# PolarisRisingWar/rgb-experiment

Measured on AMD Instinct MI355X. Metric: aggregated edges/sec (full-graph GCN d=128, reference epoch = train fwd+bwd+Adam + 2 eval fwd), higher is better.
Workload: dtype f32

## Files before the change

rgb_experiment_amd/csrc/gemm.hip:

```cpp
#include "rgbx_common.h"

namespace rgbx {
namespace {

constexpr int BM = 128, BN = 128, KT = 32;
enum { A_PLAIN = 0, A_BN = 1, A_ROWS = 2 };

struct TnExtra {
  const float* X;
  int64_t ldx;
  const float *mean, *rstd, *ca, *cb, *ck;
  const int32_t* rows;
  int64_t n_rows;
};
using f32x16 = __attribute__((ext_vector_type(16))) float;

template <int W>
__device__ __forceinline__ void stage_tile(float* __restrict__ lds, const float* __restrict__ src,
                                           int64_t ld, int64_t k0, int64_t k_end, int c0, int ncols) {
  const int tid = threadIdx.x;
#pragma unroll 4
  for (int p = 0; p < KT * W / 256; ++p) {
    const int idx = p * 256 + tid;
    const int r = idx / W, c = idx % W;
    const int64_t k = k0 + r;
    lds[r * W + c] = (k < k_end && c0 + c < ncols) ? src[k * ld + c0 + c] : 0.f;
  }
}

template <int W>
__device__ __forceinline__ void fetch_tile(float4 (&regs)[KT * (W / 4) / 256], const float* __restrict__ src, int64_t ld,
                                           int64_t k0, int64_t k_end, int c0, int ncols) {
#pragma unroll
  for (int p = 0; p < KT * (W / 4) / 256; ++p) {
    const int idx = p * 256 + threadIdx.x;
    const int r = idx / (W / 4), c = (idx % (W / 4)) * 4;
    const int64_t k = k0 + r;
    regs[p] = make_float4(0.f, 0.f, 0.f, 0.f);
    if (k < k_end && c0 + c < ncols) regs[p] = *reinterpret_cast<const float4*>(src + k * ld + c0 + c);
  }
}

template <int W>
__device__ __forceinline__ void put_tile(float* __restrict__ lds, const float4 (&regs)[KT * (W / 4) / 256]) {
#pragma unroll
  for (int p = 0; p < KT * (W / 4) / 256; ++p) {
    const int idx = p * 256 + threadIdx.x;
    const int r = idx / (W / 4), c = (idx % (W / 4)) * 4;
    *reinterpret_cast<float4*>(lds + r * W + c) = regs[p];
  }
}

template <int W>
__device__ __forceinline__ void put_tile_bn(float* __restrict__ lds, const float4 (&rg)[KT * (W / 4) / 256],
                                            const float4 (&rx)[KT * (W / 4) / 256], const float* __restrict__ lc,
                                            int64_t k0, int64_t k_end, int c0, int ncols) {
#pragma unroll
  for (int p = 0; p < KT * (W / 4) / 256; ++p) {
    const int idx = p * 256 + threadIdx.x;
    const int r = idx / (W / 4), c = (idx % (W / 4)) * 4;
    float4 v = rg[p];
    if (k0 + r < k_end && c0 + c < ncols) {
      const float4 mu = *reinterpret_cast<const float4*>(lc + 0 * W + c);
      const float4 rs = *reinterpret_cast<const float4*>(lc + 1 * W + c);
      const float4 a = *reinterpret_cast<const float4*>(lc + 2 * W + c);
      const float4 b = *reinterpret_cast<const float4*>(lc + 3 * W + c);
      const float4 k = *reinterpret_cast<const float4*>(lc + 4 * W + c);
      v.x = bn_bwd_input_grad(v.x, rx[p].x, mu.x, rs.x, a.x, b.x, k.x);
      v.y = bn_bwd_input_grad(v.y, rx[p].y, mu.y, rs.y, a.y, b.y, k.y);
      v.z = bn_bwd_input_grad(v.z, rx[p].z, mu.z, rs.z, a.z, b.z, k.z);
      v.w = bn_bwd_input_grad(v.w, rx[p].w, mu.w, rs.w, a.w, b.w, k.w);
    }
    *reinterpret_cast<float4*>(lds + r * W + c) = v;
  }
}

template <int W>
__device__ __forceinline__ void fetch_row_ids(int32_t (&ids)[KT * (W / 4) / 256], const int32_t* __restrict__ rows,
                                              int64_t j0, int64_t j_end) {
#pragma unroll
  for (int p = 0; p < KT * (W / 4) / 256; ++p) {
    const int64_t j = j0 + (p * 256 + (int)threadIdx.x) / (W / 4);
    ids[p] = j < j_end ? rows[j] : -1;
  }
}

template <int W>
__device__ __forceinline__ void fetch_tile_rows(float4 (&regs)[KT * (W / 4) / 256], const float* __restrict__ src,
                                                int64_t ld, const int32_t (&ids)[KT * (W / 4) / 256], int c0, int ncols) {
#pragma unroll
  for (int p = 0; p < KT * (W / 4) / 256; ++p) {
    const int c = ((p * 256 + (int)threadIdx.x) % (W / 4)) * 4;
    regs[p] = make_float4(0.f, 0.f, 0.f, 0.f);
    if (ids[p] >= 0 && c0 + c < ncols) regs[p] = *reinterpret_cast<const float4*>(src + (int64_t)ids[p] * ld + c0 + c);
  }
}

__device__ __forceinline__ int64_t lower_bound_rows(const int32_t* __restrict__ rows, int64_t n, int64_t key) {
  int64_t lo = 0, hi = n;
  while (lo < hi) {
    const int64_t mid = (lo + hi) >> 1;
    if (rows[mid] < key) lo = mid + 1; else hi = mid;
  }
  return lo;
}

template <bool VEC4, int MT, int MODE = A_PLAIN>
__global__ void __launch_bounds__(256)
gemm_tn_partial_kernel(const float* __restrict__ A, int64_t lda, const float* __restrict__ B, int64_t ldb,
                       float* __restrict__ part, float* __restrict__ colpart, int64_t K, int M, int N,
                       int64_t slab, TnExtra ex) {
  static_assert(MODE == A_PLAIN || VEC4, "the A_BN / A_ROWS forms exist on the 16-byte path only");
  constexpr int MI = MT / 64;
  __shared__ float lds[KT * (MT + 128) + (MODE == A_BN ? 5 * MT : 0)];
  float* la = lds;
  float* lb = lds + KT * MT;
  const int split = blockIdx.x;
  const int m0 = blockIdx.y * MT, n0 = blockIdx.z * BN;
  const int64_t k_begin = (int64_t)split * slab;
  const int64_t k_end = k_begin + slab < K ? k_begin + slab : K;
  const int wave = threadIdx.x >> 6, lane = threadIdx.x & 63;
  const int wm = (wave >> 1) * (MT / 2), wn = (wave & 1) * 64;
  const int kr = lane >> 5, cc = lane & 31;

  f32x16 acc[MI][2];
#pragma unroll
  for (int i = 0; i < MI; ++i)
#pragma unroll
    for (int j = 0; j < 2; ++j)
#pragma unroll
      for (int r = 0; r < 16; ++r) acc[i][j][r] = 0.f;

  const bool sums = colpart != nullptr && blockIdx.z == 0 && threadIdx.x < MT;
  float csum = 0.f;
  auto consume = [&]() {
    if (sums) {
#pragma unroll 8
      for (int r = 0; r < KT; ++r) csum += la[r * MT + threadIdx.x];
    }
#pragma unroll 4
    for (int kk = 0; kk < KT; kk += 2) {
      float a[MI];
#pragma unroll
      for (int i = 0; i < MI; ++i) a[i] = la[(kk + kr) * MT + wm + i * 32 + cc];
      const float b0 = lb[(kk + kr) * 128 + wn + cc];
      const float b1 = lb[(kk + kr) * 128 + wn + 32 + cc];
#pragma unroll
      for (int i = 0; i < MI; ++i) {
        acc[i][0] = __builtin_amdgcn_mfma_f32_32x32x2f32(a[i], b0, acc[i][0], 0, 0, 0);
        acc[i][1] = __builtin_amdgcn_mfma_f32_32x32x2f32(a[i], b1, acc[i][1], 0, 0, 0);
      }
    }
  };
  if constexpr (MODE == A_BN) {
    float* lc = lds + KT * (MT + 128);
    for (int i = threadIdx.x; i < 5 * MT; i += 256) {
      const float* src = i < MT ? ex.mean : i < 2 * MT ? ex.rstd : i < 3 * MT ? ex.ca : i < 4 * MT ? ex.cb : ex.ck;
      const int c = m0 + i % MT;
      lc[i] = c < M ? src[c] : 0.f;
    }
    float4 ra[KT * (MT / 4) / 256], rx[KT * (MT / 4) / 256], rb[KT * 32 / 256];
    fetch_tile<MT>(ra, A, lda, k_begin, k_end, m0, M);
    fetch_tile<MT>(rx, ex.X, ex.ldx, k_begin, k_end, m0, M);
    fetch_tile<128>(rb, B, ldb, k_begin, k_end, n0, N);
    for (int64_t k0 = k_begin; k0 < k_end; k0 += KT) {
      __syncthreads();
      put_tile_bn<MT>(la, ra, rx, lc, k0, k_end, m0, M);
      put_tile<128>(lb, rb);
      __syncthreads();
      if (k0 + KT < k_end) {
        fetch_tile<MT>(ra, A, lda, k0 + KT, k_end, m0, M);
        fetch_tile<MT>(rx, ex.X, ex.ldx, k0 + KT, k_end, m0, M);
        fetch_tile<128>(rb, B, ldb, k0 + KT, k_end, n0, N);
      }
      consume();
    }
  } else if constexpr (MODE == A_ROWS) {
    const int64_t j_begin = lower_bound_rows(ex.rows, ex.n_rows, k_begin);
    const int64_t j_end = lower_bound_rows(ex.rows, ex.n_rows, k_end);
    float4 ra[KT * (MT / 4) / 256], rb[KT * 32 / 256];
    int32_t ia[KT * (MT / 4) / 256], ib[KT * 32 / 256];
    fetch_row_ids<MT>(ia, ex.rows, j_begin, j_end);
    fetch_row_ids<128>(ib, ex.rows, j_begin, j_end);
    fetch_tile_rows<MT>(ra, A, lda, ia, m0, M);
    fetch_tile_rows<128>(rb, B, ldb, ib, n0, N);
    fetch_row_ids<MT>(ia, ex.rows, j_begin + KT, j_end);
    fetch_row_ids<128>(ib, ex.rows, j_begin + KT, j_end);
    for (int64_t j0 = j_begin; j0 < j_end; j0 += KT) {
      __syncthreads();
      put_tile<MT>(la, ra);
      put_tile<128>(lb, rb);
      __syncthreads();
      if (j0 + KT < j_end) {
        fetch_tile_rows<MT>(ra, A, lda, ia, m0, M);
        fetch_tile_rows<128>(rb, B, ldb, ib, n0, N);
        fetch_row_ids<MT>(ia, ex.rows, j0 + 2 * KT, j_end);
        fetch_row_ids<128>(ib, ex.rows, j0 + 2 * KT, j_end);
      }
      consume();
    }
  } else if constexpr (VEC4) {
    float4 ra[KT * (MT / 4) / 256], rb[KT * 32 / 256];
    fetch_tile<MT>(ra, A, lda, k_begin, k_end, m0, M);
    fetch_tile<128>(rb, B, ldb, k_begin, k_end, n0, N);
    for (int64_t k0 = k_begin; k0 < k_end; k0 += KT) {
      __syncthreads();
      put_tile<MT>(la, ra);
      put_tile<128>(lb, rb);
      __syncthreads();
      if (k0 + KT < k_end) {
        fetch_tile<MT>(ra, A, lda, k0 + KT, k_end, m0, M);
        fetch_tile<128>(rb, B, ldb, k0 + KT, k_end, n0, N);
      }
      consume();
    }
  } else {
    for (int64_t k0 = k_begin; k0 < k_end; k0 += KT) {
      __syncthreads();
      stage_tile<MT>(la, A, lda, k0, k_end, m0, M);
      stage_tile<128>(lb, B, ldb, k0, k_end, n0, N);
      __syncthreads();
      consume();
    }
  }

  if (sums && m0 + (int)threadIdx.x < M) colpart[(int64_t)split * M + m0 + threadIdx.x] = csum;
  float* out = part + (int64_t)split * M * N;
#pragma unroll
  for (int i = 0; i < MI; ++i)
#pragma unroll
    for (int j = 0; j < 2; ++j)
#pragma unroll
      for (int r = 0; r < 16; ++r) {
        const int m = m0 + wm + i * 32 + (r & 3) + 8 * (r >> 2) + 4 * kr;
        const int n = n0 + wn + j * 32 + cc;
        if (m < M && n < N) out[(int64_t)m * N + n] = acc[i][j][r];
      }
}

__global__ void __launch_bounds__(256)
gemm_tn_reduce_kernel(const float* __restrict__ part, int S, int64_t MN, float* __restrict__ C, int N,
                      int64_t ldc, float alpha) {
  __shared__ float sh[8][32];
  const int j = threadIdx.x & 31, q = threadIdx.x >> 5;
  for (int64_t base = (int64_t)blockIdx.x * 32; base < MN; base += (int64_t)gridDim.x * 32) {
    const int64_t i = base + j;
    float s = 0.f;
    if (i < MN)
      for (int p = q; p < S; p += 8) s += part[(int64_t)p * MN + i];
    __syncthreads();
    sh[q][j] = s;
    __syncthreads();
    if (q == 0 && i < MN) {
      float t = 0.f;
#pragma unroll
      for (int k = 0; k < 8; ++k) t += sh[k][j];
      C[(i / N) * ldc + (i % N)] = alpha * t;
    }
  }
}

int tile_rows(int M) { return M <= 64 ? 64 : BM; }

int choose_splits(int64_t K, int M, int N) {
  const int64_t tiles = cdiv(M, tile_rows(M)) * cdiv(N, BN);
  int64_t s = cdiv(tile_rows(M) == 64 ? 1024 : 768, tiles);
  const int64_t max_s = cdiv(K, 16 * KT);
  if (s > max_s) s = max_s;
  if (s < 1) s = 1;
  return (int)s;
}

}
}

using namespace rgbx;

extern "C" int rgbx_gemm_tn_workspace_bytes(int64_t K, int64_t M, int64_t N, size_t* bytes) {
  if (!bytes || K < 0 || M < 0 || N < 0) return fail(RGBX_E_ARG, "gemm_tn_workspace_bytes: bad argument");
  if (M >= INT32_MAX || N >= INT32_MAX) return fail(RGBX_E_RANGE, "gemm_tn: M or N exceeds int32");
  *bytes = (size_t)choose_splits(K, (int)M, (int)N) * ((size_t)M * (size_t)N + (size_t)M) * sizeof(float);
  return RGBX_OK;
}

namespace rgbx {
namespace {

int run_gemm_tn(const char* name, int mode, const float* A, int64_t lda, const float* B, int64_t ldb, float* C,
                int64_t ldc, float* a_colsum, int64_t K, int64_t M, int64_t N, float alpha, void* workspace,
                size_t workspace_bytes, rgbx_stream_t stream, const TnExtra& ex) {
  if (K < 0 || M < 0 || N < 0) return fail(RGBX_E_ARG, "%s: negative size", name);
  if (M == 0 || N == 0) return RGBX_OK;
  if (!C || (K > 0 && (!A || !B))) return fail(RGBX_E_ARG, "%s: null pointer", name);
  if (M >= INT32_MAX || N >= INT32_MAX) return fail(RGBX_E_RANGE, "%s: M or N exceeds int32", name);
  if (lda < M || ldb < N || ldc < N) return fail(RGBX_E_ARG, "%s: leading dimension too small", name);
  bool v4 = aligned16(A) && aligned16(B) && lda % 4 == 0 && ldb % 4 == 0;
  if (mode == A_BN) {
    if (K > 0 && (!ex.X || !ex.mean || !ex.rstd || !ex.ca || !ex.cb || !ex.ck))
      return fail(RGBX_E_ARG, "%s: null pointer", name);
    if (ex.ldx < M) return fail(RGBX_E_ARG, "%s: leading dimension too small", name);
    v4 = v4 && aligned16(ex.X) && ex.ldx % 4 == 0;
  }
  if (mode == A_ROWS) {
    if (ex.n_rows < 0 || ex.n_rows > K || (ex.n_rows > 0 && !ex.rows)) return fail(RGBX_E_ARG, "%s: bad row list", name);
    if (K >= INT32_MAX) return fail(RGBX_E_RANGE, "%s: K exceeds int32", name);
  }
  if (mode != A_PLAIN && !v4)
    return fail(RGBX_E_ALIGN, "%s: operands must be 16-byte aligned with leading dimensions that are multiples of 4", name);
  size_t need = 0;
  if (int rc = rgbx_gemm_tn_workspace_bytes(K, M, N, &need)) return rc;
  if (!workspace || workspace_bytes < need)
    return fail(RGBX_E_WS, "%s: workspace %zu < %zu bytes", name, workspace_bytes, need);
  hipStream_t s = (hipStream_t)stream;
  const int S = choose_splits(K, (int)M, (int)N);
  const int64_t slab = cdiv(cdiv(K > 0 ? K : 1, S), KT) * KT;
  float* part = static_cast<float*>(workspace);
  float* colpart = a_colsum ? part + (size_t)S * M * N : nullptr;
  const int mt = tile_rows((int)M);
  dim3 grid(S, (unsigned)cdiv(M, mt), (unsigned)cdiv(N, BN));
#define RGBX_GEMM_TN(V4, MT, MODE) \
  gemm_tn_partial_kernel<V4, MT, MODE><<<grid, 256, 0, s>>>(A, lda, B, ldb, part, colpart, K, (int)M, (int)N, slab, ex)
  if (mode == A_BN) { if (mt == 64) RGBX_GEMM_TN(true, 64, A_BN); else RGBX_GEMM_TN(true, 128, A_BN); }
  else if (mode == A_ROWS) { if (mt == 64) RGBX_GEMM_TN(true, 64, A_ROWS); else RGBX_GEMM_TN(true, 128, A_ROWS); }
  else if (v4) { if (mt == 64) RGBX_GEMM_TN(true, 64, A_PLAIN); else RGBX_GEMM_TN(true, 128, A_PLAIN); }
  else { if (mt == 64) RGBX_GEMM_TN(false, 64, A_PLAIN); else RGBX_GEMM_TN(false, 128, A_PLAIN); }
#undef RGBX_GEMM_TN
  RGBX_CHECK_LAUNCH("gemm_tn_partial_kernel");
  const int64_t MN = M * N;
  int64_t rb = cdiv(MN, 32);
  if (rb > kMaxGrid) rb = kMaxGrid;
  gemm_tn_reduce_kernel<<<(int)rb, 256, 0, s>>>(part, S, MN, C, (int)N, ldc, alpha);
  RGBX_CHECK_LAUNCH("gemm_tn_reduce_kernel");
  if (a_colsum) {
    gemm_tn_reduce_kernel<<<(int)cdiv(M, 32), 256, 0, s>>>(colpart, S, M, a_colsum, (int)M, M, 1.0f);
    RGBX_CHECK_LAUNCH("gemm_tn_reduce_kernel");
  }
  return RGBX_OK;
}

}
}

extern "C" int rgbx_gemm_tn_f32(const float* A, int64_t lda, const float* B, int64_t ldb, float* C,
                                int64_t ldc, float* a_colsum, int64_t K, int64_t M, int64_t N, float alpha,
                                void* workspace, size_t workspace_bytes, rgbx_stream_t stream) {
  return run_gemm_tn("gemm_tn", A_PLAIN, A, lda, B, ldb, C, ldc, a_colsum, K, M, N, alpha, workspace, workspace_bytes,
                     stream, TnExtra{});
}

extern "C" int rgbx_gemm_tn_bn_bwd_f32(const float* G, int64_t ldg, const float* X, int64_t ldx, const float* mean,
                                       const float* rstd, const float* ca, const float* cb, const float* ck,
                                       const float* B, int64_t ldb, float* C, int64_t ldc, float* a_colsum, int64_t K,
                                       int64_t M, int64_t N, float alpha, void* workspace, size_t workspace_bytes,
                                       rgbx_stream_t stream) {
  TnExtra ex{};
  ex.X = X, ex.ldx = ldx, ex.mean = mean, ex.rstd = rstd, ex.ca = ca, ex.cb = cb, ex.ck = ck;
  return run_gemm_tn("gemm_tn_bn_bwd", A_BN, G, ldg, B, ldb, C, ldc, a_colsum, K, M, N, alpha, workspace,
                     workspace_bytes, stream, ex);
}

extern "C" int rgbx_gemm_tn_rows_f32(const float* A, int64_t lda, const float* B, int64_t ldb, const int32_t* rows,
                                     int64_t n_rows, float* C, int64_t ldc, float* a_colsum, int64_t K, int64_t M,
                                     int64_t N, float alpha, void* workspace, size_t workspace_bytes,
                                     rgbx_stream_t stream) {
  TnExtra ex{};
  ex.rows = rows, ex.n_rows = n_rows;
  return run_gemm_tn("gemm_tn_rows", A_ROWS, A, lda, B, ldb, C, ldc, a_colsum, K, M, N, alpha, workspace,
                     workspace_bytes, stream, ex);
}
```

Baseline: 16.88 billion.

## Fuse colsum reduce into main reduce, batch split loads, wave-parallel row search

```diff
diff --git a/rgb_experiment_amd/csrc/gemm.hip b/rgb_experiment_amd/csrc/gemm.hip
--- a/rgb_experiment_amd/csrc/gemm.hip
+++ b/rgb_experiment_amd/csrc/gemm.hip
@@ -96,13 +96,29 @@
   }
 }
 
-__device__ __forceinline__ int64_t lower_bound_rows(const int32_t* __restrict__ rows, int64_t n, int64_t key) {
-  int64_t lo = 0, hi = n;
-  while (lo < hi) {
-    const int64_t mid = (lo + hi) >> 1;
-    if (rows[mid] < key) lo = mid + 1; else hi = mid;
-  }
-  return lo;
+__device__ __forceinline__ void lower_bound_rows_pair(const int32_t* __restrict__ rows, int64_t n, int64_t key0,
+                                                      int64_t key1, int64_t& pos0, int64_t& pos1) {
+  const int lane = threadIdx.x & 63;
+  int64_t lo[2] = {0, 0}, hi[2] = {n, n};
+  const int64_t key[2] = {key0, key1};
+  while (lo[0] < hi[0] || lo[1] < hi[1]) {
+    int64_t step[2], idx[2];
+    bool below[2];
+#pragma unroll
+    for (int t = 0; t < 2; ++t) {
+      step[t] = (hi[t] - lo[t] + 63) >> 6;
+      idx[t] = lo[t] + (lane + 1) * step[t] - 1;
+      below[t] = step[t] > 0 && idx[t] < hi[t] && rows[idx[t]] < key[t];
+    }
+#pragma unroll
+    for (int t = 0; t < 2; ++t) {
+      const int64_t c = __popcll(__ballot(below[t]));
+      const int64_t top = lo[t] + (c + 1) * step[t] - 1;
+      lo[t] += c * step[t];
+      if (step[t] > 0 && top < hi[t]) hi[t] = top;
+    }
+  }
+  pos0 = __builtin_amdgcn_readfirstlane((int)lo[0]), pos1 = __builtin_amdgcn_readfirstlane((int)lo[1]);
 }
 
 template <bool VEC4, int MT, int MODE = A_PLAIN>
@@ -176,8 +192,8 @@
       consume();
     }
   } else if constexpr (MODE == A_ROWS) {
-    const int64_t j_begin = lower_bound_rows(ex.rows, ex.n_rows, k_begin);
-    const int64_t j_end = lower_bound_rows(ex.rows, ex.n_rows, k_end);
+    int64_t j_begin, j_end;
+    lower_bound_rows_pair(ex.rows, ex.n_rows, k_begin, k_end, j_begin, j_end);
     float4 ra[KT * (MT / 4) / 256], rb[KT * 32 / 256];
     int32_t ia[KT * (MT / 4) / 256], ib[KT * 32 / 256];
     fetch_row_ids<MT>(ia, ex.rows, j_begin, j_end);
@@ -238,24 +254,38 @@
       }
 }
 
+constexpr int RU = 32;
 __global__ void __launch_bounds__(256)
 gemm_tn_reduce_kernel(const float* __restrict__ part, int S, int64_t MN, float* __restrict__ C, int N,
-                      int64_t ldc, float alpha) {
+                      int64_t ldc, float alpha, const float* __restrict__ colpart, int M,
+                      float* __restrict__ colsum, int blocks_c) {
   __shared__ float sh[8][32];
   const int j = threadIdx.x & 31, q = threadIdx.x >> 5;
-  for (int64_t base = (int64_t)blockIdx.x * 32; base < MN; base += (int64_t)gridDim.x * 32) {
+  const bool col = (int)blockIdx.x >= blocks_c;
+  const float* __restrict__ src = col ? colpart : part;
+  const int64_t n = col ? M : MN;
+  const int64_t first = col ? blockIdx.x - blocks_c : blockIdx.x, stride = col ? gridDim.x - blocks_c : blocks_c;
+  for (int64_t base = first * 32; base < n; base += stride * 32) {
     const int64_t i = base + j;
     float s = 0.f;
-    if (i < MN)
-      for (int p = q; p < S; p += 8) s += part[(int64_t)p * MN + i];
+    if (i < n)
+      for (int p0 = q; p0 < S; p0 += 8 * RU) {
+        float v[RU];
+#pragma unroll
+        for (int u = 0; u < RU; ++u) v[u] = p0 + 8 * u < S ? src[(int64_t)(p0 + 8 * u) * n + i] : 0.f;
+#pragma unroll
+        for (int u = 0; u < RU; ++u)
+          if (p0 + 8 * u < S) s += v[u];
+      }
     __syncthreads();
     sh[q][j] = s;
     __syncthreads();
-    if (q == 0 && i < MN) {
+    if (q == 0 && i < n) {
       float t = 0.f;
 #pragma unroll
       for (int k = 0; k < 8; ++k) t += sh[k][j];
-      C[(i / N) * ldc + (i % N)] = alpha * t;
+      if (col) colsum[i] = t;
+      else C[(i / N) * ldc + (i % N)] = alpha * t;
     }
   }
 }
@@ -329,12 +359,11 @@
   const int64_t MN = M * N;
   int64_t rb = cdiv(MN, 32);
   if (rb > kMaxGrid) rb = kMaxGrid;
-  gemm_tn_reduce_kernel<<<(int)rb, 256, 0, s>>>(part, S, MN, C, (int)N, ldc, alpha);
+  int64_t cb = a_colsum ? cdiv(M, 32) : 0;
+  if (cb > kMaxGrid) cb = kMaxGrid;
+  gemm_tn_reduce_kernel<<<(int)(rb + cb), 256, 0, s>>>(part, S, MN, C, (int)N, ldc, alpha, colpart, (int)M, a_colsum,
+                                                       (int)rb);
   RGBX_CHECK_LAUNCH("gemm_tn_reduce_kernel");
-  if (a_colsum) {
-    gemm_tn_reduce_kernel<<<(int)cdiv(M, 32), 256, 0, s>>>(colpart, S, M, a_colsum, (int)M, M, 1.0f);
-    RGBX_CHECK_LAUNCH("gemm_tn_reduce_kernel");
-  }
   return RGBX_OK;
 }
 
```

Measured after the change: 16.94 billion (median of 3 runs). Within noise of the previous version (+0.3%).
